# SilverlightningY/dmmt-jpeg-encoder

Measured on AMD Instinct MI355X. Metric: Mpixel/s encoded (4K PPM, q=90), higher is better.
Workload: dtype f32; 1 GPU; 3840x2160 synthetic RGB u8, 4:4:4, IJG quality 90, 1 frame(s) per step per GPU, pixels in HBM -> JPEG files in HBM, inputs rotating over 12 distinct slots (285 MiB: streamed from HBM); width=3840, height=2160, subsampling=P444, quality=90, parallelism=independent frames x1, lanes=4, input_slots=12

## Files before the change

dmmt-jpeg-encoder_amd/csrc/coef_format.hpp:

```cpp
#pragma once
#include <stdint.h>

#include "jpeg_common.hpp"

namespace dmmt {

constexpr int kCoefLoCount = 8;
constexpr int kCoefLoBytes = 2 * kCoefLoCount, kCoefHiBytes = 64;
constexpr int kCoefEscape = -128;

constexpr bool coef_in_lo(int k) { return k < kCoefLoCount; }
constexpr int coef_hi_byte(int v) { return v < -127 || v > 127 ? kCoefEscape : v; }
constexpr int coef_hi_word(int k) { return coef_pos(k) >> 2; }
constexpr int coef_hi_shift(int k) { return 8 * (coef_pos(k) & 3); }
constexpr int coef_lo_rows(int c) { return c == 0 ? 3 : c < 3 ? 2 : c == 3 ? 1 : 0; }

inline void coef_pack_block(const int16_t* zz, int16_t* lo, int8_t* hi, int16_t* wide) {
    for (int k = 0; k < kCoefLoCount; ++k) lo[k] = zz[k];
    bool esc[8] = {false};
    bool any = false;
    for (int k = 0; k < 64; ++k) {
        const int p = coef_pos(k);
        const int b = coef_in_lo(k) ? 0 : coef_hi_byte(zz[k]);
        hi[p] = (int8_t)b;
        if (!coef_in_lo(k) && b == kCoefEscape) esc[p >> 3] = any = true;
    }
    hi[coef_pos(0)] = any ? 1 : 0;
    for (int k = 0; k < 64; ++k)
        if (esc[coef_pos(k) >> 3]) wide[coef_pos(k)] = zz[k];
}
inline bool coef_block_flag(const int8_t* hi) { return hi[coef_pos(0)] != 0; }
inline int coef_read(int k, const int16_t* lo, const int8_t* hi, const int16_t* wide) {
    if (coef_in_lo(k)) return lo[k];
    const int b = hi[coef_pos(k)];
    return coef_block_flag(hi) && b == kCoefEscape ? wide[coef_pos(k)] : b;
}

enum { COEF_FORMAT_AUTO = 0, COEF_FORMAT_WIDE = 1, COEF_FORMAT_NARROW = 2 };
constexpr int kCoefNarrowMinQ = 2;
inline bool coef_narrow_for(int mode, int sample_bytes, const uint8_t* luma_q, const uint8_t* chroma_q) {
    if (sample_bytes == 4 || mode == COEF_FORMAT_WIDE) return false;
    if (mode == COEF_FORMAT_NARROW) return true;
    for (int k = kCoefLoCount; k < 64; ++k)
        if (luma_q[kZigzag[k]] < kCoefNarrowMinQ || chroma_q[kZigzag[k]] < kCoefNarrowMinQ) return false;
    return true;
}

#ifdef __HIPCC__
__device__ __forceinline__ bool coef_word_escapes(uint32_t w) {
    const uint32_t t = w ^ 0x80808080u;
    return ((t - 0x01010101u) & ~t & 0x80808080u) != 0u;
}

__device__ __forceinline__ void coef_store_column_narrow(const int (&x)[8], int col, int el, bool valid,
                                                         int16_t* __restrict__ wide, int16_t* __restrict__ lo,
                                                         int8_t* __restrict__ hi) {
    uint32_t c[8];
#pragma unroll
    for (int i = 0; i < 8; ++i) c[i] = (uint32_t)min(max(x[i], -128), 128);
    uint32_t w0 = __builtin_amdgcn_perm(c[1], c[0], 0x0c0c0400u) | __builtin_amdgcn_perm(c[3], c[2], 0x04000c0cu);
    const uint32_t w1 = __builtin_amdgcn_perm(c[5], c[4], 0x0c0c0400u) | __builtin_amdgcn_perm(c[7], c[6], 0x04000c0cu);
    w0 &= 0xFFFFFFFFu << (8 * (col == 0 ? 3 : col < 3 ? 2 : col == 3 ? 1 : 0));
    const uint32_t p = __builtin_amdgcn_perm((uint32_t)x[1], (uint32_t)x[0], 0x05040100u);
    const uint32_t s1 = (uint32_t)__builtin_amdgcn_update_dpp(0, (int)p, 0x101, 0xF, 0xF, true);
    const uint32_t s2 = (uint32_t)__builtin_amdgcn_update_dpp(0, (int)p, 0x102, 0xF, 0xF, true);
    const uint32_t s3 = (uint32_t)__builtin_amdgcn_update_dpp(0, (int)p, 0x103, 0xF, 0xF, true);
    const bool esc = coef_word_escapes(w0) || coef_word_escapes(w1);
    const unsigned long long em = __builtin_amdgcn_ballot_w64(esc);
    if (em != 0) {
        const uint32_t lane = __builtin_amdgcn_mbcnt_hi(~0u, __builtin_amdgcn_mbcnt_lo(~0u, 0u));
        const uint32_t group = (uint32_t)(em >> (lane & 56u)) & 0xFFu;
        w0 |= col == 0 && group != 0u ? 1u : 0u;
    }
    if (valid) {
        *reinterpret_cast<uint2*>(hi + (el * 64 + 8 * col)) = make_uint2(w0, w1);
        if (col == 0) {
            const uint32_t l0 = __builtin_amdgcn_perm(s1, p, 0x05040100u);
            const uint32_t l1 = __builtin_amdgcn_perm((uint32_t)x[2], p, 0x05040302u);
            const uint32_t l2 = __builtin_amdgcn_perm(s2, s1, 0x05040302u);
            const uint32_t l3 = __builtin_amdgcn_perm(s2, s3, 0x07060100u);
            *reinterpret_cast<uint4*>(lo + el * 8) = make_uint4(l0, l1, l2, l3);
        }
        if (esc) {
            uint32_t pk[4];
            pk[0] = p;
#pragma unroll
            for (int i = 1; i < 4; ++i) pk[i] = __builtin_amdgcn_perm((uint32_t)x[2 * i + 1], (uint32_t)x[2 * i], 0x05040100u);
            *reinterpret_cast<uint4*>(wide + (el * 64 + 8 * col)) = make_uint4(pk[0], pk[1], pk[2], pk[3]);
        }
    }
}

struct NarrowCoef {
    uint32_t lo[4];
    uint32_t hi[16];
};
__device__ __forceinline__ void load_narrow(const int16_t* __restrict__ lo, const int8_t* __restrict__ hi, long long e,
                                            NarrowCoef& b) {
    const uint4 l = *reinterpret_cast<const uint4*>(lo + e * 8);
    b.lo[0] = l.x, b.lo[1] = l.y, b.lo[2] = l.z, b.lo[3] = l.w;
    const uint4* q = reinterpret_cast<const uint4*>(hi + e * 64);
#pragma unroll
    for (int i = 0; i < 4; ++i) {
        const uint4 v = q[i];
        b.hi[4 * i] = v.x, b.hi[4 * i + 1] = v.y, b.hi[4 * i + 2] = v.z, b.hi[4 * i + 3] = v.w;
// ... 11 lines not shown
```

dmmt-jpeg-encoder_amd/csrc/dct_quant.hpp:

```cpp
#pragma once
#ifdef __HIPCC__
#include <hip/hip_runtime.h>
#define DMMT_DQ_FN __device__ __forceinline__
#define DMMT_DQ_FRACT(a) __builtin_amdgcn_fractf(a)
#else
#include <math.h>
#define DMMT_DQ_FN inline
#define DMMT_DQ_FRACT(a) ((a) - floorf(a))
#endif
#include <stdint.h>

#ifndef DMMT_QUANT_F32_BAND
#define DMMT_QUANT_F32_BAND 0x1p-20f
#endif
#ifndef DMMT_QUANT_SCALED_BAND
#define DMMT_QUANT_SCALED_BAND 0x1p-21f
#endif
#ifndef DMMT_QUANT_SCALED_HALF
#define DMMT_QUANT_SCALED_HALF 0.49999905f
#endif
#ifndef DMMT_QUANT_ON_REDO
#define DMMT_QUANT_ON_REDO(r) ((void)0)
#endif

// ... 55 lines not shown
    const float v24 = (-v14) - v15, v25 = v15 + v16, v26 = v16 + v17;
    const float v30 = v20 + v21, v31 = v20 - v21, v32 = v22 + v23;
    const float v42 = v32 * DMMT_A1;
    const float v44 = ((-v24) * DMMT_A2) - ((v24 + v26) * DMMT_A5);
    const float v45 = v25 * DMMT_A3;
    const float v46 = (v26 * DMMT_A4) - ((v26 + v24) * DMMT_A5);
    const float v52 = v42 + v23, v53 = v23 - v42, v55 = v45 + v17, v57 = v17 - v45;
    const float v64 = v44 + v57, v65 = v55 + v46, v66 = v55 - v46, v67 = v57 - v44;
    v[0] = v30;
    v[4] = v31;
    v[2] = v52;
    v[6] = v53;
    v[5] = v64;
    v[1] = v65;
    v[7] = v66;
    v[3] = v67;
}

DMMT_DQ_FN void arai8(float (&v)[8]) {
    arai8_unscaled(v);
    v[0] = v[0] * DMMT_S0;
    v[1] = v[1] * DMMT_S1;
    v[2] = v[2] * DMMT_S2;
    v[3] = v[3] * DMMT_S3;
    v[4] = v[4] * DMMT_S4;
    v[5] = v[5] * DMMT_S5;
    v[6] = v[6] * DMMT_S6;
    v[7] = v[7] * DMMT_S7;
}

DMMT_DQ_FN float quant_margin(float t, float n) {
    return __builtin_fmaf(fabsf(t), DMMT_QUANT_SCALED_BAND, fabsf(t - n));
}
DMMT_DQ_FN void quantize_col8_scaled(const float (&u)[8], const float* q, const float* crq, bool nan_possible,
                                     int (&x)[8]) {
    float dist = 0.0f;
#pragma unroll
    for (int r = 0; r < 8; ++r) {
        const float t = u[r] * crq[8 * r];
        const float n = __builtin_rintf(t);
        dist = fmaxf(dist, quant_margin(t, n));
        x[r] = (int)n;
    }
    if (nan_possible || !(dist < DMMT_QUANT_SCALED_HALF)) {
#pragma unroll
        for (int r = 0; r < 8; ++r) {
            const float t = u[r] * crq[8 * r];
            if (!(quant_margin(t, __builtin_rintf(t)) < DMMT_QUANT_SCALED_HALF)) {
                DMMT_QUANT_ON_REDO(r);
                x[r] = quantize(u[r] * c_arai_scale[r], q[8 * r]);
            }
        }
    }
}

}
```

dmmt-jpeg-encoder_amd/csrc/device_common.hpp:

```cpp
#pragma once
#include <hip/hip_runtime.h>
#include <stdint.h>

namespace dmmt {

#ifdef DMMT_PHASE_TRACE
#define DMMT_TRACE_START                                                  \
    unsigned long long _dmmt_tr = __builtin_amdgcn_s_memrealtime();       \
    const unsigned long long _dmmt_t0 = _dmmt_tr;                         \
    unsigned long long _dmmt_tc = __builtin_amdgcn_s_memtime();           \
    unsigned long long _dmmt_acc[16], _dmmt_clk[16];                      \
    unsigned _dmmt_cnt[16];                                               \
    _Pragma("unroll") for (int _i = 0; _i < 16; ++_i) {                   \
        _dmmt_acc[_i] = 0;                                                \
        _dmmt_clk[_i] = 0;                                                \
        _dmmt_cnt[_i] = 0;                                                \
    }
#define DMMT_TRACE(i)                                                     \
    do {                                                                  \
        const unsigned long long _n = __builtin_amdgcn_s_memrealtime();   \
        const unsigned long long _c = __builtin_amdgcn_s_memtime();       \
        _dmmt_acc[(i) & 15] += _n - _dmmt_tr;                             \
        _dmmt_clk[(i) & 15] += _c - _dmmt_tc;                             \
        _dmmt_cnt[(i) & 15] += 1;                                         \
// ... 2 lines not shown
    } while (0)
#ifndef DMMT_TRACE_TID
#define DMMT_TRACE_TID 0
#endif
#define DMMT_TRACE_FLUSH(base, span)                                      \
    do {                                                                  \
        if (threadIdx.x == DMMT_TRACE_TID) {                              \
            const unsigned long long _e = __builtin_amdgcn_s_memrealtime(); \
            atomicMax(&g_trace[48 + 4 * (span)], ~_dmmt_t0);              \
            atomicMax(&g_trace[49 + 4 * (span)], _e);                     \
            atomicAdd(&g_trace[50 + 4 * (span)], _e - _dmmt_t0);          \
            atomicAdd(&g_trace[51 + 4 * (span)], 1ull);                   \
            _Pragma("unroll") for (int _i = 0; _i < 16; ++_i) if (_dmmt_cnt[_i]) { \
                atomicAdd(&g_trace[(base) + _i], _dmmt_acc[_i]);          \
                atomicAdd(&g_trace[16 + (base) + _i], _dmmt_clk[_i]);     \
                atomicAdd(&g_trace[32 + (base) + _i], (unsigned long long)_dmmt_cnt[_i]); \
            }                                                             \
        }                                                                 \
    } while (0)
#else
#define DMMT_TRACE_START \
    do {                 \
    } while (0)
#define DMMT_TRACE(i) \
    do {              \
    } while (0)
#define DMMT_TRACE_FLUSH(base, span) \
    do {                       \
    } while (0)
#endif

__device__ __forceinline__ int lane_id() { return threadIdx.x & 63; }

__device__ __forceinline__ uint32_t wave_sum_u32(uint32_t v) {
#pragma unroll
    for (int d = 32; d > 0; d >>= 1) v += __shfl_xor(v, d, 64);
    return v;
}

__device__ __forceinline__ uint32_t wave_sum_full_u32(uint32_t v) {
    v += (uint32_t)__builtin_amdgcn_update_dpp(0, (int)v, 0xB1, 0xF, 0xF, false);
    v += (uint32_t)__builtin_amdgcn_update_dpp(0, (int)v, 0x4E, 0xF, 0xF, false);
    v += (uint32_t)__builtin_amdgcn_update_dpp(0, (int)v, 0x141, 0xF, 0xF, false);
    v += (uint32_t)__builtin_amdgcn_update_dpp(0, (int)v, 0x140, 0xF, 0xF, false);
    return (uint32_t)__builtin_amdgcn_readlane((int)v, 0) + (uint32_t)__builtin_amdgcn_readlane((int)v, 16) +
           (uint32_t)__builtin_amdgcn_readlane((int)v, 32) + (uint32_t)__builtin_amdgcn_readlane((int)v, 48);
}

__device__ __forceinline__ uint32_t lane_prev_u32(uint32_t v) {
    return (uint32_t)__builtin_amdgcn_update_dpp(0, (int)v, 0x138, 0xF, 0xF, true);
}
__device__ __forceinline__ uint32_t lane_next_u32(uint32_t v) {
    return (uint32_t)__builtin_amdgcn_update_dpp(0, (int)v, 0x130, 0xF, 0xF, true);
}

__device__ __forceinline__ uint32_t wave_incl_scan_full_u32(uint32_t v) {
    const int s = (int)v;
    int x = s;
    x += __builtin_amdgcn_update_dpp(0, s, 0x111, 0xF, 0xF, true);
    x += __builtin_amdgcn_update_dpp(0, s, 0x112, 0xF, 0xF, true);
    x += __builtin_amdgcn_update_dpp(0, s, 0x113, 0xF, 0xF, true);
    x += __builtin_amdgcn_update_dpp(0, x, 0x114, 0xF, 0xE, true);
    x += __builtin_amdgcn_update_dpp(0, x, 0x118, 0xF, 0xC, true);
    x += __builtin_amdgcn_update_dpp(0, x, 0x142, 0xA, 0xF, false);
    x += __builtin_amdgcn_update_dpp(0, x, 0x143, 0xC, 0xF, false);
    return (uint32_t)x;
// ... 110 lines not shown
```

dmmt-jpeg-encoder_amd/csrc/entropy.hip:

```cpp
#include <hip/hip_runtime.h>
#include <stdint.h>

#include "device_common.hpp"
#include "jpeg_common.hpp"
#include "kernels.hpp"
#include "slot_copy.hpp"

namespace dmmt {

#ifdef DMMT_PHASE_TRACE
static __device__ unsigned long long g_trace[64];
#endif

static_assert(kChunkBlocks == 256 || kChunkBlocks == 512, "one thread per block, one workgroup per chunk");
constexpr int kEmitThreads = kChunkBlocks;
constexpr int kEmitWaves = kEmitThreads / 64;
#ifndef DMMT_EMIT_OCC
#define DMMT_EMIT_OCC 8
#endif
constexpr int kEmitOcc = kChunkBlocks == 256 ? DMMT_EMIT_OCC : 3;
#ifndef DMMT_EMIT_OCC_BATCH
#define DMMT_EMIT_OCC_BATCH 7
#endif
constexpr int kEmitOccBatch = kChunkBlocks == 256 ? DMMT_EMIT_OCC_BATCH : 3;

constexpr int kEmitWords = 4 * kChunkBlocks;
constexpr int kStuffPass = 4096;
#ifndef DMMT_EMIT_BRANCHFREE
#define DMMT_EMIT_BRANCHFREE 1
#endif
#ifndef DMMT_TAIL_DMA
#define DMMT_TAIL_DMA 1
#endif
#ifndef DMMT_TAIL_NSEG1
#define DMMT_TAIL_NSEG1 1
#endif
#ifndef DMMT_WALK_COLUMN_MAJOR
#define DMMT_WALK_COLUMN_MAJOR 1
#endif
#ifndef DMMT_EMIT_PRIO_ALWAYS
#define DMMT_EMIT_PRIO_ALWAYS 0
#endif
#ifndef DMMT_EMIT_PRIO
#define DMMT_EMIT_PRIO 1
#endif

struct ChunkSpan {
    long long el0;
    int nb;
    int seg;
    bool seg_first, seg_last;
};

__device__ __forceinline__ ChunkSpan chunk_span(const Geom& g, int c) {
    ChunkSpan r;
    r.seg = min(c / g.cps, g.nseg - 1);
    const int j = c - r.seg * g.cps;
    const long long sb = (long long)r.seg * g.seg_blocks;
    const long long se = min(sb + g.seg_blocks, g.bpf);
    r.el0 = sb + (long long)j * kChunkBlocks;
    r.nb = (int)min((long long)kChunkBlocks, se - r.el0);
    r.seg_first = j == 0;
    r.seg_last = r.el0 + r.nb == se;
    return r;
}

__device__ __forceinline__ bool joined_tail(const Geom& g, int c) {
    return c == g.nch - 1 && g.more_after && g.restart_interval == 0;
// ... 803 lines not shown
#pragma unroll
        for (int i = 0; i < KP; ++i) {
            const int c = c0 + i;
            if (c >= c1) continue;
            bit0[c] = b0[i];
            outo[c] = orun;
            orun += ob[i];
        }
        if (tid == 0) total_out[frame] = tot;
        return;
    }

    bool f = false;
    unsigned long long v = 0;
    for (int c = c0; c < c1; ++c)
        seg_combine(f, v, chunk_span(g, c).seg_first, cbits[c] + (c == 0 ? (unsigned long long)g.bit_phase : 0ull));
    unsigned long long run = block_segscan_1024(f, v, sWave, sWaveF);
    unsigned long long mine = 0;
    for (int c = c0; c < c1; ++c) {
        if (chunk_span(g, c).seg_first) run = c == 0 ? (unsigned long long)g.bit_phase : 0ull;
        bit0[c] = run;
        mine += chunk_out_bytes(cff, cbits, cedge, g, c, run);
        run += cbits[c];
    }
    unsigned long long tot = 0;
    unsigned long long orun = block_scan_1024(mine, sWave, &tot);
    for (int c = c0; c < c1; ++c) {
        outo[c] = orun;
        orun += chunk_out_bytes(cff, cbits, cedge, g, c, bit0[c]);
    }
    if (tid == 0) total_out[frame] = tot;
}

__global__ __launch_bounds__(256, 8) void k_stuffwrite(const uint32_t* __restrict__ stage,
                                                    const uint32_t* __restrict__ chunk_bits,
                                                    const uint32_t* __restrict__ chunk_edge,
                                                    const unsigned long long* __restrict__ chunk_bit0,
                                                    const unsigned long long* __restrict__ chunk_out,
                                                    const unsigned long long* __restrict__ total_out,
                                                    const uint32_t* __restrict__ hdr_len, Geom g,
                                                    uint8_t* __restrict__ out, size_t out_stride,
                                                    uint32_t* __restrict__ out_len, int* __restrict__ status) {
    __shared__ uint32_t sWave[4];
    __shared__ __attribute__((aligned(16))) uint8_t sOut[2 * kStuffPass + 16];
    const int tid = threadIdx.x, lane = lane_id(), wave = tid >> 6;
    const int frame = blockIdx.y;
    const int c = blockIdx.x;
    const size_t cid = (size_t)frame * g.nch + c;
    const bool last = c == g.nch - 1;
    const size_t cidn = last ? cid : cid + 1;
    const uint32_t hdr = hdr_len[frame];
    const unsigned long long tot = total_out[frame];
    const unsigned long long b0 = chunk_bit0[cid];
    const uint32_t n = chunk_bits[cid], edge = chunk_edge[cid];
    const uint32_t n_next = chunk_bits[cidn], edge_next = chunk_edge[cidn];
    const unsigned long long cout = chunk_out[cid], cout_next = chunk_out[cidn];
    const uint32_t* slot = stage + cid * (size_t)kChunkWordsCap;
    uint32_t wv0[5];
    {
        const uint4 q = *reinterpret_cast<const uint4*>(slot + 4 * tid);
        wv0[0] = q.x, wv0[1] = q.y, wv0[2] = q.z, wv0[3] = q.w;
        wv0[4] = slot[4 * tid + 4];
    }
    asm volatile("" ::"s"(hdr), "s"(tot), "s"(b0), "s"(n), "s"(edge), "s"(n_next), "s"(edge_next), "s"(cout),
                 "s"(cout_next), "v"(wv0[0]), "v"(wv0[1]), "v"(wv0[2]), "v"(wv0[3]), "v"(wv0[4]));
    const unsigned long long end = (unsigned long long)hdr + tot;
// ... 27 lines not shown
            const unsigned long long at = (last ? tot : cout_next) - 2;
            base[at] = 0xFF;
            base[at + 1] = (uint8_t)(0xD0 + ((g.seg_base + sp.seg) & 7));
            if (last) out_len[frame] = (uint32_t)end;
        } else if (last) {
            out_len[frame] = (uint32_t)end;
        }
    }
    const unsigned long long e = b0 + n;
    const unsigned long long kbeg = (b0 + 7) >> 3, kend = (e + 7) >> 3;
    if (kend <= kbeg) return;
    const unsigned long long nbytes = kend - kbeg;
    const bool shared_tail = (e & 7) != 0;
    uint32_t tail = 0;
    if (shared_tail) {
        const bool jt = joined_tail(g, c);
        const bool has_next = !sp.seg_last || jt;
        tail = boundary_byte((int)(e & 7), edge & 0xFFFFu, has_next,
                             jt ? (uint32_t)g.next_bits : (has_next ? n_next : 0u),
                             jt ? g.next16 : (has_next ? edge_next >> 16 : 0u));
    }
    const unsigned off = (unsigned)(8 * kbeg - b0);
    uint8_t* o = base + cout;
    for (unsigned long long pos = 0; pos < nbytes; pos += kStuffPass) {
        const uint32_t delta = (uint32_t)(reinterpret_cast<uintptr_t>(o) & 15u);
        const unsigned long long kb = pos + 16u * (unsigned)tid;
        const int nvalid = kb < nbytes ? (int)min(16ull, nbytes - kb) : 0;
        uint32_t x[4] = {0u, 0u, 0u, 0u};
        uint32_t ffm[4] = {0u, 0u, 0u, 0u};
        uint32_t cnt = 0;
        if (nvalid) {
            const unsigned long long p = off + 8 * kb;
            const size_t wi = (size_t)(p >> 5);
            const int sh = (int)(p & 31);
            uint32_t wv[5];
#pragma unroll
            for (int i = 0; i < 5; ++i) wv[i] = pos ? slot[wi + i] : wv0[i];
#pragma unroll
            for (int i = 0; i < 4; ++i) x[i] = sh ? (wv[i] << sh) | (wv[i + 1] >> (32 - sh)) : wv[i];
            if (shared_tail && nbytes - 1 - kb < 16) {
                const int j = (int)(nbytes - 1 - kb), sft = 24 - 8 * (j & 3);
                x[j >> 2] = (x[j >> 2] & ~(0xFFu << sft)) | (tail << sft);
            }
#pragma unroll
            for (int i = 0; i < 4; ++i) {
                const int nv = min(max(nvalid - 4 * i, 0), 4);
                const uint32_t vmask = nv ? 0x80808080u & (0xFFFFFFFFu << (32 - 8 * nv)) : 0u;
                const uint32_t t = ~x[i];
                const uint32_t nonzero = (((t & 0x7F7F7F7Fu) + 0x7F7F7F7Fu) | t) & 0x80808080u;
                ffm[i] = ~nonzero & vmask;
                cnt += (uint32_t)__popc(ffm[i]);
            }
        }
        const uint32_t incl = wave_incl_scan_full_u32(cnt);
        if (lane == 63) sWave[wave] = incl;
        __syncthreads();
        uint32_t pre = incl - cnt;
        for (int q = 0; q < wave; ++q) pre += sWave[q];
        const uint32_t ffs = sWave[0] + sWave[1] + sWave[2] + sWave[3];
        if (nvalid) {
            const uint32_t dst = delta + (uint32_t)tid * 16u + pre;
            uint32_t a = dst;
#pragma unroll
            for (int i = 0; i < 4; ++i) {
                const uint32_t w = x[i], f = ffm[i];
                sOut[a + 4 * i] = (uint8_t)(w >> 24);
                sOut[a + (uint32_t)__popc(f & 0x80000000u) + 4 * i + 1] = (uint8_t)(w >> 16);
                sOut[a + (uint32_t)__popc(f & 0x80800000u) + 4 * i + 2] = (uint8_t)(w >> 8);
                sOut[a + (uint32_t)__popc(f & 0x80808000u) + 4 * i + 3] = (uint8_t)w;
                a += (uint32_t)__popc(f);
            }
            if (cnt) {
                uint32_t m = 0;
#pragma unroll
                for (int i = 0; i < 4; ++i)
                    m |= ((((ffm[i] >> 7) * 0x08040201u) >> 24) & 0xFu) << (4 * i);
                uint32_t z = dst + 1;
                while (m) {
                    sOut[z + (uint32_t)__builtin_ctz(m)] = 0x00;
                    ++z;
                    m &= m - 1u;
                }
            }
        }
        __syncthreads();
        const unsigned long long in_pass = nbytes - pos < (unsigned long long)kStuffPass ? nbytes - pos : kStuffPass;
        const uint32_t len = (uint32_t)in_pass + ffs;
        const uint32_t send = delta + len;
        uint8_t* const oa = o - delta;
        for (uint32_t sb = 16u * (uint32_t)tid; sb + 16u <= send; sb += 16u * 256u) {
            if (sb >= delta) *reinterpret_cast<uint4*>(oa + sb) = *reinterpret_cast<const uint4*>(sOut + sb);
        }
        if (tid < 32) {
            const uint32_t sbt = send & ~15u;
            const uint32_t i = tid < 16 ? (uint32_t)tid : sbt + (uint32_t)tid - 16u;
            const bool mine = tid < 16 ? i >= delta && (delta > 0u || send < 16u) : sbt > 0u;
            if (mine && i < send) oa[i] = sOut[i];
        }
        o += len;
        __syncthreads();
    }
}

bool offsets_fusable(const Geom& g) { return g.nch <= kFusedOffsetsMaxChunks; }

hipError_t launch_emit(int n_frames, const Geom& g, const Work& w, bool fuse_offsets, hipStream_t st, bool prio) {
    const int fuse = fuse_offsets && offsets_fusable(g) ? 1 : 0;
    if (w.coef_lo) {
        const auto kn = !prio && n_frames > 1 ? k_emit_n<kEmitOccBatch> : k_emit_n<kEmitOcc>;
        hipLaunchKernelGGL(kn, dim3(g.nch, n_frames), dim3(kEmitThreads), 0, st, (const int16_t*)w.coef,
                           (const int16_t*)w.coef_lo, (const int8_t*)w.coef_hi, (const int16_t*)w.dcdiff,
                           (const uint8_t*)w.lastnz, (const uint32_t*)w.code_tab, g, w.stage, w.chunk_bits, w.chunk_ff,
                           w.chunk_edge, w.ac_hist, w.dc_hist, fuse, w.arrive, w.chunk_bit0, w.chunk_out, w.total_out,
                           w.chunk_ff8, prio || DMMT_EMIT_PRIO_ALWAYS ? 1 : 0);
        return hipGetLastError();
    }
    const auto kern = !prio && n_frames > 1 ? k_emit<kEmitOccBatch> : k_emit<kEmitOcc>;
    hipLaunchKernelGGL(kern, dim3(g.nch, n_frames), dim3(kEmitThreads), 0, st, (const int16_t*)w.coef,
                       (const int16_t*)w.dcdiff, (const uint8_t*)w.lastnz, (const uint32_t*)w.code_tab, g, w.stage, w.chunk_bits, w.chunk_ff,
                       w.chunk_edge, w.ac_hist, w.dc_hist, fuse, w.arrive, w.chunk_bit0, w.chunk_out, w.total_out,
                       w.chunk_ff8, prio || DMMT_EMIT_PRIO_ALWAYS ? 1 : 0);
    return hipGetLastError();
}

hipError_t launch_offsets(int n_frames, const Geom& g, const Work& w, hipStream_t st) {
    hipLaunchKernelGGL(k_offsets, dim3(n_frames), dim3(1024), 0, st, (const uint32_t*)w.chunk_bits,
                       (const uint32_t*)w.chunk_ff, (const uint32_t*)w.chunk_edge, g, w.chunk_bit0, w.chunk_out,
                       w.total_out);
    return hipGetLastError();
}

hipError_t launch_stuffwrite(int n_frames, const Geom& g, const Work& w, uint8_t* out, size_t out_stride,
                             uint32_t* out_len, hipStream_t st) {
    hipLaunchKernelGGL(k_stuffwrite, dim3(g.nch, n_frames), dim3(256), 0, st, (const uint32_t*)w.stage,
                       (const uint32_t*)w.chunk_bits, (const uint32_t*)w.chunk_edge,
                       (const unsigned long long*)w.chunk_bit0, (const unsigned long long*)w.chunk_out,
                       (const unsigned long long*)w.total_out, (const uint32_t*)w.hdr_len, g, out, out_stride,
                       out_len, w.status);
    return hipGetLastError();
}

}

#ifdef DMMT_PHASE_TRACE
extern "C" int dmmt_debug_trace_entropy(unsigned long long* out64) {
    if (hipMemcpyFromSymbol(out64, HIP_SYMBOL(dmmt::g_trace), 64 * 8) != hipSuccess) return -1;
    unsigned long long z[64] = {0};
    return hipMemcpyToSymbol(HIP_SYMBOL(dmmt::g_trace), z, sizeof z) == hipSuccess ? 0 : -1;
}
#endif
```

dmmt-jpeg-encoder_amd/csrc/front_common.hpp:

```cpp
#pragma once
#include <hip/hip_runtime.h>
#include <stdint.h>

#include "coef_format.hpp"
#include "dct_quant.hpp"
#include "device_common.hpp"
#include "jpeg_common.hpp"

namespace dmmt {

template <int HR_, int VR_, int NCOMP_ = 3>
struct FrontGeom {
    static_assert(NCOMP_ == 3 || (NCOMP_ == 1 && HR_ == 1 && VR_ == 1), "gray: one block per MCU");
    static constexpr int HR = HR_, VR = VR_, NCOMP = NCOMP_;
    static constexpr int TM = 32 / HR;
    static constexpr int ROWS = 8 * VR;
    static constexpr int NLUMA = HR * VR;
    static constexpr int BPM = NLUMA + NCOMP - 1;
    static constexpr int NB = TM * BPM;
    static constexpr int NYB = 32 * VR;
    static constexpr int CB = NCOMP == 1 ? 0 : TM;
    static constexpr int NQT = NCOMP == 1 ? 1 : 2;
    static constexpr int BS = 72;
    static constexpr int ST_FLOATS = NB * BS + 4;
// ... 46 lines not shown
    uint32_t t[N + 1];
#pragma unroll
    for (int i = 0; i <= N; ++i) t[i] = a[i];
#pragma unroll
    for (int i = 0; i < N; ++i) o[i] = __builtin_amdgcn_alignbyte(t[i + 1], t[i], (uint32_t)off & 3u);
}

template <int NCHUNK, int NQ>
__device__ __forceinline__ void front_stage(uint8_t* sRaw, int tid, const uint4 (&v)[NQ]) {
    static_assert(NQ == (NCHUNK + 255) / 256, "chunks per thread");
#pragma unroll
    for (int i = 0; i < NQ; ++i) {
        const int q = tid + 256 * i;
        if (q < NCHUNK) reinterpret_cast<uint4*>(sRaw)[q] = v[i];
    }
}

template <class G, bool SCALED>
__device__ __forceinline__ void front_fill_qtabs(const float* __restrict__ qtab,
                                                 float* sQ, float* sRQ, int tid) {
    if (tid < 64 * G::NQT) sQ[tid] = qtab[tid];
    if (tid < 64 * G::NQT) sRQ[tid] = SCALED ? c_arai_scale[(tid >> 3) & 7] * (1.0f / qtab[tid]) : 1.0f / qtab[tid];
}

template <class G, bool NARROW, bool F32>
__device__ __forceinline__ void front_column_pass(const float* sT, const float* sQ, const float* sRQ, int tid,
                                                  bool nan_possible, const Geom& g, int frame, int mx0, int my,
                                                  int16_t* coef, int16_t* coef_lo, int8_t* coef_hi) {
    static_assert(!NARROW || !F32, "Image<f32> dots are unbounded: wide blocks");
    const int col = tid & 7;
    const int nvalid = min(G::TM, g.mcux - mx0) * G::BPM;
    const long long e0 = (long long)frame * g.bpf + ((long long)my * g.mcux + mx0) * G::BPM;
    int16_t* const cbase = coef + e0 * 64;
#pragma unroll
    for (int jj = 0; jj < G::JPT; ++jj) {
        const int blk = (tid + 256 * jj) >> 3;
        int x[8];
        {
            const int qt = G::NQT == 1 || blk < G::NYB ? 0 : 64;
            const float* q = sQ + qt + col;
            const float* rq = sRQ + qt + col;
            float v[8];
            const float* tb = sT + G::blk_base(blk) + col;
#pragma unroll
            for (int i = 0; i < 8; ++i) v[i] = tb[i * 8];
            if constexpr (F32) {
                arai8(v);
                quantize_col8(v, q, rq, x);
            } else {
                arai8_unscaled(v);
                quantize_col8_scaled(v, q, rq, nan_possible, x);
            }
        }
        const int el = G::NCOMP == 1 ? blk : G::emit_index(blk);
        const bool valid = el < nvalid;
        if constexpr (NARROW) {
            coef_store_column_narrow(x, col, el, valid, cbase, coef_lo + e0 * 8, coef_hi + e0 * 64);
        } else if (valid) {
            uint32_t pk[4];
#pragma unroll
            for (int i = 0; i < 4; ++i) pk[i] = __builtin_amdgcn_perm((uint32_t)x[2 * i + 1], (uint32_t)x[2 * i], 0x05040100u);
            *reinterpret_cast<uint4*>(cbase + (el * 64 + 8 * col)) = make_uint4(pk[0], pk[1], pk[2], pk[3]);
        }
    }
}

}
```

dmmt-jpeg-encoder_amd/csrc/kernels.hip:

```cpp

#include <hip/hip_runtime.h>
#include <stdint.h>
#include <stdlib.h>

#include <type_traits>

#include "dct_quant.hpp"
#include "device_common.hpp"
#include "front_common.hpp"
#include "front_launch.hpp"
#include "jpeg_common.hpp"
#include "kernels.hpp"
#include "surface_load.hpp"
#include "wave_merge.hpp"

namespace dmmt {

#ifdef DMMT_PHASE_TRACE
static __device__ unsigned long long g_trace[64];
#endif

__constant__ uint8_t c_zigzag[64] = {0,  1,  8,  16, 9,  2,  3,  10, 17, 24, 32, 25, 18, 11, 4,  5,
                                     12, 19, 26, 33, 40, 48, 41, 34, 27, 20, 13, 6,  7,  14, 21, 28,
                                     35, 42, 49, 56, 57, 50, 43, 36, 29, 22, 15, 23, 30, 37, 44, 51,
// ... 956 lines not shown
    uint32_t* ct = code_tab + ((size_t)frame * 4 + tab) * 256;
    {
        const int rk = n - 1 - s;
        const uint32_t wgt = sym_thread && s < n ? 1u << (16 - sLen[rk]) : 0u;
        const uint32_t incl = wave_incl_scan_full_u32(wgt);
        if (sym_thread && lane == 63) sWave[wave] = incl;
        __syncthreads();
        uint32_t excl = incl - wgt;
        for (int q = 0; q < wave; ++q) excl += sWave[q];
        if (sym_thread && f == 0) ct[s] = 0;
        __syncthreads();
        if (sym_thread && s < n) {
            const int L = sLen[rk];
            const uint32_t pat = excl & 0xFFFFu;
            ct[sSym[rk]] = ((uint32_t)L << 16) | (pat >> (16 - L));
        }
    }
    DMMT_TRACE(14);

    if (!sym_thread) return;
    write_table_header(out + (size_t)frame * out_stride, tab, s, 256, n, nt, sSym, sBits, g, qtab_u8, bits_per_channel,
                       hdr_len + frame);
    DMMT_TRACE(15);
    DMMT_TRACE_FLUSH(0, 1);
}

#ifndef DMMT_TAIL_SORT2
#define DMMT_TAIL_SORT2 1
#endif
constexpr int kTailLevels = 15;
constexpr int kTailBase[4] = {0, 208, 3536, 3744};
static_assert(kTailBase[3] + 3328 == kTailLdsBytes, "tables_tail's LDS regions");

__device__ __forceinline__ void wave_lds_sync() {
    __builtin_amdgcn_fence(__ATOMIC_SEQ_CST, "wavefront");
    __builtin_amdgcn_wave_barrier();
}

template <int EPL>
__device__ __forceinline__ void tail_levels(const uint32_t* F, int n, int (&leaf)[kTailLevels]) {
    const int lane = lane_id();
    constexpr int H = EPL == 1 ? 1 : EPL / 2;
    auto leaf_index = [&](int t) { return EPL == 1 ? lane : 64 * t + lane; };
    auto pkg_index = [&](int t) { return EPL == 1 ? 63 - lane : 32 * EPL - 1 - 64 * t - lane; };
    uint32_t lk[H], pk[H];
    int np = n >> 1;
#pragma unroll
    for (int t = 0; t < H; ++t) {
        const int i = leaf_index(t), j = pkg_index(t);
        lk[t] = i < n ? F[min(i, 255)] << 1 : kMergeInf;
        pk[t] = j >= 0 && j < np ? ((F[2 * j] + F[2 * j + 1]) << 1) | 1u : kMergeInf;
    }
    uint32_t mlo[2] = {0u, 0u}, mhi[2] = {0u, 0u}, mcum[2] = {0u, 0u};
    const int src = 8 * (31 - (lane & 31));
    for (int k = 1; k < kTailLevels; ++k) {
        uint32_t x[EPL];
        if constexpr (EPL == 1) {
            x[0] = lane < 32 ? lk[0] : pk[0];
        } else {
#pragma unroll
            for (int t = 0; t < H; ++t) {
                x[t] = lk[t];
                x[H + t] = pk[t];
            }
        }
        merge_bitonic<EPL>(x);
        int before = 0;
#pragma unroll
        for (int s = 0; s < EPL; ++s) {
            const unsigned long long m = __ballot((x[s] & 1u) != 0u);
            const int e = k * EPL + s;
// ... 456 lines not shown
```

Baseline: 207,200 Mpixel/s.

## Stuff each entropy chunk with one wave and fold escape detection into quantize

Rewrites the byte-stuffing/write kernel so each wavefront handles one chunk in 1 KiB passes with wave-level scans and wave-local LDS sync instead of block-wide __syncthreads and cross-wave prefix sums. It prefetches the first few passes into registers and launches four chunks per workgroup. It also adds an optional path (off by default) that computes the narrow-coefficient escape test from float magnitudes during quantization, skipping the clamp when no lane escapes. The stuffing change trades block-level parallelism per chunk for less synchronisation, and may lengthen per-chunk latency for large chunks.

```diff
diff --git a/dmmt-jpeg-encoder_amd/csrc/coef_format.hpp b/dmmt-jpeg-encoder_amd/csrc/coef_format.hpp
--- a/dmmt-jpeg-encoder_amd/csrc/coef_format.hpp
+++ b/dmmt-jpeg-encoder_amd/csrc/coef_format.hpp
@@ -47,30 +47,77 @@
 }
 
 #ifdef __HIPCC__
+#define DMMT_CF_FN __host__ __device__ __forceinline__
+#else
+#define DMMT_CF_FN inline
+#endif
+DMMT_CF_FN float coef_hi_mag_row(float m, int r, float n, int c) {
+    static_assert(coef_lo_rows(0) == 3 && coef_lo_rows(1) == 2 && coef_lo_rows(2) == 2 && coef_lo_rows(3) == 1 &&
+                      coef_lo_rows(4) == 0 && coef_lo_rows(7) == 0,
+                  "row 2 is hi from column 1 on, row 1 from column 3 on, row 0 from column 4 on");
+    const float a = __builtin_fabsf(n);
+    const bool hi = r >= 3 || c >= (r == 0 ? 4 : r == 1 ? 3 : 1);
+    return __builtin_fmaxf(m, hi ? a : 0.0f);
+}
+DMMT_CF_FN float coef_hi_mag(const float (&n)[8], int c) {
+    float m = 0.0f;
+    for (int r = 0; r < 8; ++r) m = coef_hi_mag_row(m, r, n[r], c);
+    return m;
+}
+constexpr float kCoefHiMagMax = 127.0f;
+inline bool coef_column_escapes(const int16_t* x, int c) {
+    float n[8];
+    for (int r = 0; r < 8; ++r) n[r] = (float)x[r];
+    return coef_hi_mag(n, c) > kCoefHiMagMax;
+}
+
+#ifndef DMMT_NARROW_FOLD
+#define DMMT_NARROW_FOLD 0
+#endif
+
+#ifdef __HIPCC__
 __device__ __forceinline__ bool coef_word_escapes(uint32_t w) {
     const uint32_t t = w ^ 0x80808080u;
     return ((t - 0x01010101u) & ~t & 0x80808080u) != 0u;
 }
 
-__device__ __forceinline__ void coef_store_column_narrow(const int (&x)[8], int col, int el, bool valid,
+template <bool FOLD>
+__device__ __forceinline__ void coef_store_column_narrow(const int (&x)[8], bool esc_fold, int col, int el, bool valid,
                                                          int16_t* __restrict__ wide, int16_t* __restrict__ lo,
                                                          int8_t* __restrict__ hi) {
-    uint32_t c[8];
-#pragma unroll
-    for (int i = 0; i < 8; ++i) c[i] = (uint32_t)min(max(x[i], -128), 128);
-    uint32_t w0 = __builtin_amdgcn_perm(c[1], c[0], 0x0c0c0400u) | __builtin_amdgcn_perm(c[3], c[2], 0x04000c0cu);
-    const uint32_t w1 = __builtin_amdgcn_perm(c[5], c[4], 0x0c0c0400u) | __builtin_amdgcn_perm(c[7], c[6], 0x04000c0cu);
-    w0 &= 0xFFFFFFFFu << (8 * (col == 0 ? 3 : col < 3 ? 2 : col == 3 ? 1 : 0));
+    auto pack4 = [](uint32_t a, uint32_t b, uint32_t c, uint32_t d) {
+        return __builtin_amdgcn_perm(b, a, 0x0c0c0400u) | __builtin_amdgcn_perm(d, c, 0x04000c0cu);
+    };
+    const uint32_t himask = 0xFFFFFFFFu << (8 * (col == 0 ? 3 : col < 3 ? 2 : col == 3 ? 1 : 0));
     const uint32_t p = __builtin_amdgcn_perm((uint32_t)x[1], (uint32_t)x[0], 0x05040100u);
     const uint32_t s1 = (uint32_t)__builtin_amdgcn_update_dpp(0, (int)p, 0x101, 0xF, 0xF, true);
     const uint32_t s2 = (uint32_t)__builtin_amdgcn_update_dpp(0, (int)p, 0x102, 0xF, 0xF, true);
     const uint32_t s3 = (uint32_t)__builtin_amdgcn_update_dpp(0, (int)p, 0x103, 0xF, 0xF, true);
-    const bool esc = coef_word_escapes(w0) || coef_word_escapes(w1);
-    const unsigned long long em = __builtin_amdgcn_ballot_w64(esc);
-    if (em != 0) {
-        const uint32_t lane = __builtin_amdgcn_mbcnt_hi(~0u, __builtin_amdgcn_mbcnt_lo(~0u, 0u));
-        const uint32_t group = (uint32_t)(em >> (lane & 56u)) & 0xFFu;
-        w0 |= col == 0 && group != 0u ? 1u : 0u;
+    uint32_t w0, w1;
+    bool esc;
+    unsigned long long em;
+    if (FOLD) {
+        esc = esc_fold;
+        em = __builtin_amdgcn_ballot_w64(esc);
+    }
+    if (FOLD && em == 0) {
+        w0 = pack4((uint32_t)x[0], (uint32_t)x[1], (uint32_t)x[2], (uint32_t)x[3]) & himask;
+        w1 = pack4((uint32_t)x[4], (uint32_t)x[5], (uint32_t)x[6], (uint32_t)x[7]);
+    } else {
+        uint32_t c[8];
+#pragma unroll
+        for (int i = 0; i < 8; ++i) c[i] = (uint32_t)min(max(x[i], -128), 128);
+        w0 = pack4(c[0], c[1], c[2], c[3]) & himask;
+        w1 = pack4(c[4], c[5], c[6], c[7]);
+        if (!FOLD) {
+            esc = coef_word_escapes(w0) || coef_word_escapes(w1);
+            em = __builtin_amdgcn_ballot_w64(esc);
+        }
+        if (em != 0) {
+            const uint32_t lane = __builtin_amdgcn_mbcnt_hi(~0u, __builtin_amdgcn_mbcnt_lo(~0u, 0u));
+            const uint32_t group = (uint32_t)(em >> (lane & 56u)) & 0xFFu;
+            w0 |= col == 0 && group != 0u ? 1u : 0u;
+        }
     }
     if (valid) {
         *reinterpret_cast<uint2*>(hi + (el * 64 + 8 * col)) = make_uint2(w0, w1);
diff --git a/dmmt-jpeg-encoder_amd/csrc/dct_quant.hpp b/dmmt-jpeg-encoder_amd/csrc/dct_quant.hpp
--- a/dmmt-jpeg-encoder_amd/csrc/dct_quant.hpp
+++ b/dmmt-jpeg-encoder_amd/csrc/dct_quant.hpp
@@ -111,16 +111,22 @@
 DMMT_DQ_FN float quant_margin(float t, float n) {
     return __builtin_fmaf(fabsf(t), DMMT_QUANT_SCALED_BAND, fabsf(t - n));
 }
-DMMT_DQ_FN void quantize_col8_scaled(const float (&u)[8], const float* q, const float* crq, bool nan_possible,
-                                     int (&x)[8]) {
+template <bool FOLD, class Fold>
+DMMT_DQ_FN void quantize_col8_scaled_impl(const float (&u)[8], const float* q, const float* crq, bool nan_possible,
+                                          int (&x)[8], const Fold& fold, float& mag) {
     float dist = 0.0f;
+    if constexpr (FOLD) mag = 0.0f;
 #pragma unroll
     for (int r = 0; r < 8; ++r) {
         const float t = u[r] * crq[8 * r];
         const float n = __builtin_rintf(t);
         dist = fmaxf(dist, quant_margin(t, n));
         x[r] = (int)n;
+        if constexpr (FOLD) mag = fold(mag, r, n);
     }
+#ifdef __HIP_DEVICE_COMPILE__
+    if constexpr (FOLD) asm volatile("" : "+v"(mag));
+#endif
     if (nan_possible || !(dist < DMMT_QUANT_SCALED_HALF)) {
 #pragma unroll
         for (int r = 0; r < 8; ++r) {
@@ -130,7 +136,22 @@
                 x[r] = quantize(u[r] * c_arai_scale[r], q[8 * r]);
             }
         }
+        if constexpr (FOLD) {
+            mag = 0.0f;
+#pragma unroll
+            for (int r = 0; r < 8; ++r) mag = fold(mag, r, (float)x[r]);
+        }
     }
+}
+DMMT_DQ_FN void quantize_col8_scaled(const float (&u)[8], const float* q, const float* crq, bool nan_possible,
+                                     int (&x)[8]) {
+    float mag;
+    quantize_col8_scaled_impl<false>(u, q, crq, nan_possible, x, 0, mag);
+}
+template <class Fold>
+DMMT_DQ_FN void quantize_col8_scaled_fold(const float (&u)[8], const float* q, const float* crq, bool nan_possible,
+                                          int (&x)[8], const Fold& fold, float& mag) {
+    quantize_col8_scaled_impl<true>(u, q, crq, nan_possible, x, fold, mag);
 }
 
 }
diff --git a/dmmt-jpeg-encoder_amd/csrc/device_common.hpp b/dmmt-jpeg-encoder_amd/csrc/device_common.hpp
--- a/dmmt-jpeg-encoder_amd/csrc/device_common.hpp
+++ b/dmmt-jpeg-encoder_amd/csrc/device_common.hpp
@@ -58,6 +58,11 @@
 
 __device__ __forceinline__ int lane_id() { return threadIdx.x & 63; }
 
+__device__ __forceinline__ void wave_lds_sync() {
+    __builtin_amdgcn_fence(__ATOMIC_SEQ_CST, "wavefront");
+    __builtin_amdgcn_wave_barrier();
+}
+
 __device__ __forceinline__ uint32_t wave_sum_u32(uint32_t v) {
 #pragma unroll
     for (int d = 32; d > 0; d >>= 1) v += __shfl_xor(v, d, 64);
diff --git a/dmmt-jpeg-encoder_amd/csrc/entropy.hip b/dmmt-jpeg-encoder_amd/csrc/entropy.hip
--- a/dmmt-jpeg-encoder_amd/csrc/entropy.hip
+++ b/dmmt-jpeg-encoder_amd/csrc/entropy.hip
@@ -25,7 +25,6 @@
 constexpr int kEmitOccBatch = kChunkBlocks == 256 ? DMMT_EMIT_OCC_BATCH : 3;
 
 constexpr int kEmitWords = 4 * kChunkBlocks;
-constexpr int kStuffPass = 4096;
 #ifndef DMMT_EMIT_BRANCHFREE
 #define DMMT_EMIT_BRANCHFREE 1
 #endif
@@ -34,6 +33,9 @@
 #endif
 #ifndef DMMT_TAIL_NSEG1
 #define DMMT_TAIL_NSEG1 1
+#endif
+#ifndef DMMT_STUFF_WAVE_CHUNK
+#define DMMT_STUFF_WAVE_CHUNK 1
 #endif
 #ifndef DMMT_WALK_COLUMN_MAJOR
 #define DMMT_WALK_COLUMN_MAJOR 1
@@ -903,6 +905,194 @@
     if (tid == 0) total_out[frame] = tot;
 }
 
+__device__ __forceinline__ uint32_t stuff_piece(const uint32_t (&wv)[5], int sh, int nvalid, bool with_tail, int j,
+                                                uint32_t tail, uint32_t (&x)[4], uint32_t (&ffm)[4]) {
+#pragma unroll
+    for (int i = 0; i < 4; ++i) x[i] = sh ? (wv[i] << sh) | (wv[i + 1] >> (32 - sh)) : wv[i];
+    if (with_tail) {
+        const int sft = 24 - 8 * (j & 3);
+        x[j >> 2] = (x[j >> 2] & ~(0xFFu << sft)) | (tail << sft);
+    }
+    uint32_t cnt = 0;
+#pragma unroll
+    for (int i = 0; i < 4; ++i) {
+        const int nv = min(max(nvalid - 4 * i, 0), 4);
+        const uint32_t vmask = nv ? 0x80808080u & (0xFFFFFFFFu << (32 - 8 * nv)) : 0u;
+        const uint32_t t = ~x[i];
+        const uint32_t nonzero = (((t & 0x7F7F7F7Fu) + 0x7F7F7F7Fu) | t) & 0x80808080u;
+        ffm[i] = ~nonzero & vmask;
+        cnt += (uint32_t)__popc(ffm[i]);
+    }
+    return cnt;
+}
+
+__device__ __forceinline__ void stuff_stage(uint8_t* sOut, uint32_t dst, const uint32_t (&x)[4], const uint32_t (&ffm)[4],
+                                            uint32_t cnt) {
+    uint32_t a = dst;
+#pragma unroll
+    for (int i = 0; i < 4; ++i) {
+        const uint32_t w = x[i], f = ffm[i];
+        sOut[a + 4 * i] = (uint8_t)(w >> 24);
+        sOut[a + (uint32_t)__popc(f & 0x80000000u) + 4 * i + 1] = (uint8_t)(w >> 16);
+        sOut[a + (uint32_t)__popc(f & 0x80800000u) + 4 * i + 2] = (uint8_t)(w >> 8);
+        sOut[a + (uint32_t)__popc(f & 0x80808000u) + 4 * i + 3] = (uint8_t)w;
+        a += (uint32_t)__popc(f);
+    }
+    if (cnt) {
+        uint32_t m = 0;
+#pragma unroll
+        for (int i = 0; i < 4; ++i)
+            m |= ((((ffm[i] >> 7) * 0x08040201u) >> 24) & 0xFu) << (4 * i);
+        uint32_t z = dst + 1;
+        while (m) {
+            sOut[z + (uint32_t)__builtin_ctz(m)] = 0x00;
+            ++z;
+            m &= m - 1u;
+        }
+    }
+}
+
+#if DMMT_STUFF_WAVE_CHUNK
+constexpr int kStuffWavePass = 1024;
+constexpr int kStuffWaveLds = 2 * kStuffWavePass + 16;
+constexpr int kStuffPre = 4;
+static_assert(kStuffPre * (kStuffWavePass / 4) + 1 <= kChunkWordsCap, "the words read unasked lie inside the chunk's slot");
+
+__global__ __launch_bounds__(256, 8) void k_stuffwrite(const uint32_t* __restrict__ stage,
+                                                    const uint32_t* __restrict__ chunk_bits,
+                                                    const uint32_t* __restrict__ chunk_edge,
+                                                    const unsigned long long* __restrict__ chunk_bit0,
+                                                    const unsigned long long* __restrict__ chunk_out,
+                                                    const unsigned long long* __restrict__ total_out,
+                                                    const uint32_t* __restrict__ hdr_len, Geom g,
+                                                    uint8_t* __restrict__ out, size_t out_stride,
+                                                    uint32_t* __restrict__ out_len, int* __restrict__ status) {
+    __shared__ __attribute__((aligned(16))) uint8_t sAll[4 * kStuffWaveLds];
+    const int lane = lane_id();
+    const int wave = __builtin_amdgcn_readfirstlane((int)threadIdx.x >> 6);
+    const int frame = blockIdx.y;
+    const int c = 4 * (int)blockIdx.x + wave;
+    if (c >= g.nch) return;
+    uint8_t* const sOut = sAll + wave * kStuffWaveLds;
+    const size_t cid = (size_t)frame * g.nch + c;
+    const bool last = c == g.nch - 1;
+    const size_t cidn = last ? cid : cid + 1;
+    const uint32_t hdr = hdr_len[frame];
+    const unsigned long long tot = total_out[frame];
+    const unsigned long long b0 = chunk_bit0[cid];
+    const uint32_t n = chunk_bits[cid], edge = chunk_edge[cid];
+    const uint32_t n_next = chunk_bits[cidn], edge_next = chunk_edge[cidn];
+    const unsigned long long cout = chunk_out[cid], cout_next = chunk_out[cidn];
+    const uint32_t* slot = stage + cid * (size_t)kChunkWordsCap;
+    uint32_t wpre[kStuffPre][5];
+#pragma unroll
+    for (int k = 0; k < kStuffPre; ++k) {
+        const uint32_t* w = slot + (kStuffWavePass / 4) * k + 4 * lane;
+        const uint4 q = *reinterpret_cast<const uint4*>(w);
+        wpre[k][0] = q.x, wpre[k][1] = q.y, wpre[k][2] = q.z, wpre[k][3] = q.w;
+        wpre[k][4] = w[4];
+    }
+    asm volatile("" ::"s"(hdr), "s"(tot), "s"(b0), "s"(n), "s"(edge), "s"(n_next), "s"(edge_next), "s"(cout),
+                 "s"(cout_next));
+#pragma unroll
+    for (int k = 0; k < kStuffPre; ++k)
+        asm volatile("" ::"v"(wpre[k][0]), "v"(wpre[k][1]), "v"(wpre[k][2]), "v"(wpre[k][3]), "v"(wpre[k][4]));
+    const unsigned long long end = (unsigned long long)hdr + tot;
+    if (end + 2 > out_stride) {
+        if (c == 0 && lane == 0) {
+            out_len[frame] = 0;
+            raise_status(status, 16);
+        }
+        return;
+    }
+    {
+        const unsigned long long cend = last ? tot : cout_next;
+        const unsigned long long sbytes = ((unsigned long long)n + 7) / 8 + 1;
+        if (n > (uint32_t)kChunkWordsCap * 32u || cout > cend || cend > tot ||
+            (unsigned long long)hdr + cout + 2 * sbytes > out_stride) {
+            if (lane == 0) {
+                out_len[frame] = 0;
+                raise_status(status, 16);
+            }
+            return;
+        }
+    }
+    const ChunkSpan sp = chunk_span(g, c);
+    uint8_t* const base = out + (size_t)frame * out_stride + hdr;
+    if (lane == 0) {
+        if (last && !g.more_after) {
+            base[tot] = 0xFF;
+            base[tot + 1] = 0xD9;
+            out_len[frame] = (uint32_t)(end + 2);
+        } else if (sp.seg_last && g.restart_interval > 0) {
+            const unsigned long long at = (last ? tot : cout_next) - 2;
+            base[at] = 0xFF;
+            base[at + 1] = (uint8_t)(0xD0 + ((g.seg_base + sp.seg) & 7));
+            if (last) out_len[frame] = (uint32_t)end;
+        } else if (last) {
+            out_len[frame] = (uint32_t)end;
+        }
+    }
+    const unsigned long long e = b0 + n;
+    const unsigned long long kbeg = (b0 + 7) >> 3, kend = (e + 7) >> 3;
+    if (kend <= kbeg) return;
+    const uint32_t nbytes = (uint32_t)(kend - kbeg);
+    const bool shared_tail = (e & 7) != 0;
+    uint32_t tail = 0;
+    if (shared_tail) {
+        const bool jt = joined_tail(g, c);
+        const bool has_next = !sp.seg_last || jt;
+        tail = boundary_byte((int)(e & 7), edge & 0xFFFFu, has_next,
+                             jt ? (uint32_t)g.next_bits : (has_next ? n_next : 0u),
+                             jt ? g.next16 : (has_next ? edge_next >> 16 : 0u));
+    }
+    const int sh = (int)(8 * kbeg - b0);
+    uint8_t* o = base + cout;
+    auto pass = [&](uint32_t pos, const uint32_t (&wv)[5]) {
+        const uint32_t delta = (uint32_t)(reinterpret_cast<uintptr_t>(o) & 15u);
+        const uint32_t kb = pos + 16u * (uint32_t)lane;
+        const int nvalid = kb < nbytes ? (int)min(16u, nbytes - kb) : 0;
+        uint32_t x[4] = {0u, 0u, 0u, 0u};
+        uint32_t ffm[4] = {0u, 0u, 0u, 0u};
+        uint32_t cnt = 0;
+        if (nvalid) cnt = stuff_piece(wv, sh, nvalid, shared_tail && nbytes - 1 - kb < 16, (int)(nbytes - 1 - kb), tail, x, ffm);
+        const uint32_t incl = wave_incl_scan_full_u32(cnt);
+        const uint32_t ffs = (uint32_t)__builtin_amdgcn_readlane((int)incl, 63);
+        if (nvalid) stuff_stage(sOut, delta + (uint32_t)lane * 16u + (incl - cnt), x, ffm, cnt);
+        wave_lds_sync();
+        const uint32_t len = min(nbytes - pos, (uint32_t)kStuffWavePass) + ffs;
+        const uint32_t send = delta + len;
+        uint8_t* const oa = o - delta;
+        for (uint32_t sb = 16u * (uint32_t)lane; sb + 16u <= send; sb += 16u * 64u) {
+            if (sb >= delta) *reinterpret_cast<uint4*>(oa + sb) = *reinterpret_cast<const uint4*>(sOut + sb);
+        }
+        if (lane < 32) {
+            const uint32_t sbt = send & ~15u;
+            const uint32_t i = lane < 16 ? (uint32_t)lane : sbt + (uint32_t)lane - 16u;
+            const bool mine = lane < 16 ? i >= delta && (delta > 0u || send < 16u) : sbt > 0u;
+            if (mine && i < send) oa[i] = sOut[i];
+        }
+        o += len;
+        wave_lds_sync();
+    };
+#pragma unroll
+    for (int k = 0; k < kStuffPre; ++k) {
+        if ((uint32_t)(kStuffWavePass * k) >= nbytes) return;
+        pass((uint32_t)(kStuffWavePass * k), wpre[k]);
+    }
+    for (uint32_t pos = kStuffPre * kStuffWavePass; pos < nbytes; pos += kStuffWavePass) {
+        uint32_t wv[5] = {0u, 0u, 0u, 0u, 0u};
+        if (pos + 16u * (uint32_t)lane < nbytes) {
+            const uint32_t* w = slot + (pos >> 2) + 4 * lane;
+            const uint4 q = *reinterpret_cast<const uint4*>(w);
+            wv[0] = q.x, wv[1] = q.y, wv[2] = q.z, wv[3] = q.w;
+            wv[4] = w[4];
+        }
+        pass(pos, wv);
+    }
+}
+#else
+constexpr int kStuffPass = 4096;
 __global__ __launch_bounds__(256, 8) void k_stuffwrite(const uint32_t* __restrict__ stage,
                                                     const uint32_t* __restrict__ chunk_bits,
                                                     const uint32_t* __restrict__ chunk_edge,
@@ -996,25 +1186,11 @@
         if (nvalid) {
             const unsigned long long p = off + 8 * kb;
             const size_t wi = (size_t)(p >> 5);
-            const int sh = (int)(p & 31);
             uint32_t wv[5];
 #pragma unroll
             for (int i = 0; i < 5; ++i) wv[i] = pos ? slot[wi + i] : wv0[i];
-#pragma unroll
-            for (int i = 0; i < 4; ++i) x[i] = sh ? (wv[i] << sh) | (wv[i + 1] >> (32 - sh)) : wv[i];
-            if (shared_tail && nbytes - 1 - kb < 16) {
-                const int j = (int)(nbytes - 1 - kb), sft = 24 - 8 * (j & 3);
-                x[j >> 2] = (x[j >> 2] & ~(0xFFu << sft)) | (tail << sft);
-            }
-#pragma unroll
-            for (int i = 0; i < 4; ++i) {
-                const int nv = min(max(nvalid - 4 * i, 0), 4);
-                const uint32_t vmask = nv ? 0x80808080u & (0xFFFFFFFFu << (32 - 8 * nv)) : 0u;
-                const uint32_t t = ~x[i];
-                const uint32_t nonzero = (((t & 0x7F7F7F7Fu) + 0x7F7F7F7Fu) | t) & 0x80808080u;
-                ffm[i] = ~nonzero & vmask;
-                cnt += (uint32_t)__popc(ffm[i]);
-            }
+            cnt = stuff_piece(wv, (int)(p & 31), nvalid, shared_tail && nbytes - 1 - kb < 16, (int)(nbytes - 1 - kb), tail,
+                              x, ffm);
         }
         const uint32_t incl = wave_incl_scan_full_u32(cnt);
         if (lane == 63) sWave[wave] = incl;
@@ -1023,29 +1199,7 @@
         for (int q = 0; q < wave; ++q) pre += sWave[q];
         const uint32_t ffs = sWave[0] + sWave[1] + sWave[2] + sWave[3];
         if (nvalid) {
-            const uint32_t dst = delta + (uint32_t)tid * 16u + pre;
-            uint32_t a = dst;
-#pragma unroll
-            for (int i = 0; i < 4; ++i) {
-                const uint32_t w = x[i], f = ffm[i];
-                sOut[a + 4 * i] = (uint8_t)(w >> 24);
-                sOut[a + (uint32_t)__popc(f & 0x80000000u) + 4 * i + 1] = (uint8_t)(w >> 16);
-                sOut[a + (uint32_t)__popc(f & 0x80800000u) + 4 * i + 2] = (uint8_t)(w >> 8);
-                sOut[a + (uint32_t)__popc(f & 0x80808000u) + 4 * i + 3] = (uint8_t)w;
-                a += (uint32_t)__popc(f);
-            }
-            if (cnt) {
-                uint32_t m = 0;
-#pragma unroll
-                for (int i = 0; i < 4; ++i)
-                    m |= ((((ffm[i] >> 7) * 0x08040201u) >> 24) & 0xFu) << (4 * i);
-                uint32_t z = dst + 1;
-                while (m) {
-                    sOut[z + (uint32_t)__builtin_ctz(m)] = 0x00;
-                    ++z;
-                    m &= m - 1u;
-                }
-            }
+            stuff_stage(sOut, delta + (uint32_t)tid * 16u + pre, x, ffm, cnt);
         }
         __syncthreads();
         const unsigned long long in_pass = nbytes - pos < (unsigned long long)kStuffPass ? nbytes - pos : kStuffPass;
@@ -1065,6 +1219,7 @@
         __syncthreads();
     }
 }
+#endif
 
 bool offsets_fusable(const Geom& g) { return g.nch <= kFusedOffsetsMaxChunks; }
 
@@ -1096,7 +1251,8 @@
 
 hipError_t launch_stuffwrite(int n_frames, const Geom& g, const Work& w, uint8_t* out, size_t out_stride,
                              uint32_t* out_len, hipStream_t st) {
-    hipLaunchKernelGGL(k_stuffwrite, dim3(g.nch, n_frames), dim3(256), 0, st, (const uint32_t*)w.stage,
+    const int per_wg = DMMT_STUFF_WAVE_CHUNK ? 4 : 1;
+    hipLaunchKernelGGL(k_stuffwrite, dim3((g.nch + per_wg - 1) / per_wg, n_frames), dim3(256), 0, st, (const uint32_t*)w.stage,
                        (const uint32_t*)w.chunk_bits, (const uint32_t*)w.chunk_edge,
                        (const unsigned long long*)w.chunk_bit0, (const unsigned long long*)w.chunk_out,
                        (const unsigned long long*)w.total_out, (const uint32_t*)w.hdr_len, g, out, out_stride,
diff --git a/dmmt-jpeg-encoder_amd/csrc/front_common.hpp b/dmmt-jpeg-encoder_amd/csrc/front_common.hpp
--- a/dmmt-jpeg-encoder_amd/csrc/front_common.hpp
+++ b/dmmt-jpeg-encoder_amd/csrc/front_common.hpp
@@ -102,10 +102,12 @@
     const int nvalid = min(G::TM, g.mcux - mx0) * G::BPM;
     const long long e0 = (long long)frame * g.bpf + ((long long)my * g.mcux + mx0) * G::BPM;
     int16_t* const cbase = coef + e0 * 64;
+    constexpr bool FOLD = NARROW && DMMT_NARROW_FOLD;
 #pragma unroll
     for (int jj = 0; jj < G::JPT; ++jj) {
         const int blk = (tid + 256 * jj) >> 3;
         int x[8];
+        float mag = 0.0f;
         {
             const int qt = G::NQT == 1 || blk < G::NYB ? 0 : 64;
             const float* q = sQ + qt + col;
@@ -117,6 +119,9 @@
             if constexpr (F32) {
                 arai8(v);
                 quantize_col8(v, q, rq, x);
+            } else if constexpr (FOLD) {
+                arai8_unscaled(v);
+                quantize_col8_scaled_fold(v, q, rq, nan_possible, x, [&](float m, int r, float n) { return coef_hi_mag_row(m, r, n, col); }, mag);
             } else {
                 arai8_unscaled(v);
                 quantize_col8_scaled(v, q, rq, nan_possible, x);
@@ -125,7 +130,7 @@
         const int el = G::NCOMP == 1 ? blk : G::emit_index(blk);
         const bool valid = el < nvalid;
         if constexpr (NARROW) {
-            coef_store_column_narrow(x, col, el, valid, cbase, coef_lo + e0 * 8, coef_hi + e0 * 64);
+            coef_store_column_narrow<FOLD>(x, mag > kCoefHiMagMax, col, el, valid, cbase, coef_lo + e0 * 8, coef_hi + e0 * 64);
         } else if (valid) {
             uint32_t pk[4];
 #pragma unroll
diff --git a/dmmt-jpeg-encoder_amd/csrc/kernels.hip b/dmmt-jpeg-encoder_amd/csrc/kernels.hip
--- a/dmmt-jpeg-encoder_amd/csrc/kernels.hip
+++ b/dmmt-jpeg-encoder_amd/csrc/kernels.hip
@@ -1012,11 +1012,6 @@
 constexpr int kTailBase[4] = {0, 208, 3536, 3744};
 static_assert(kTailBase[3] + 3328 == kTailLdsBytes, "tables_tail's LDS regions");
 
-__device__ __forceinline__ void wave_lds_sync() {
-    __builtin_amdgcn_fence(__ATOMIC_SEQ_CST, "wavefront");
-    __builtin_amdgcn_wave_barrier();
-}
-
 template <int EPL>
 __device__ __forceinline__ void tail_levels(const uint32_t* F, int n, int (&leaf)[kTailLevels]) {
     const int lane = lane_id();
```

After: 211,100 Mpixel/s (median of 6 runs). +1.9%, better.
